# landonclark97/numbotics

Hardware: AMD Instinct MI355X
Metric: collision-checked configs/sec, Kinova 7-DoF + obstacles (higher is better)
Workload: dtype f64

## Files before the change

numbotics_amd/csrc/nbk.hip:

```cpp
#include <hip/hip_runtime.h>
#include <stdint.h>
#include <math.h>
#include <stdio.h>
#include <stdlib.h>
#include <string.h>

#include <memory>
#include <mutex>
#include <atomic>
#include <algorithm>
#include <vector>
#include <string>
#include <map>
#include <dlfcn.h>
#include <hip/hiprtc.h>

#include "../../include/nbk.h"
#include "nbk_device.hpp"
#include "nbk_bf32_common.hpp"

namespace nbk {

struct DevModel {
    int n_q, n_joints, n_rshapes, n_wshapes, n_pairs;
// ... 1138 lines not shown
    const unsigned lo = (unsigned)__builtin_amdgcn_readlane((int)(unsigned)u, l);
    const unsigned hi = (unsigned)__builtin_amdgcn_readlane((int)(unsigned)(u >> 32), l);
    return __builtin_bit_cast(double, ((unsigned long long)hi << 32) | lo);
}

constexpr int NSUB = 256;
constexpr int CNT_TICKET = 1;

struct DevRoute {
    const DevModel& m;
    NBK_DEV int cls(unsigned p) const { return m.vp_cls[p]; }
    NBK_DEV int base(int c) const { return m.cls_base[c]; }
    NBK_DEV int groups(int c) const { return m.cls_groups[c]; }
};
NBK_DEV void flush_items(const DevModel& m, unsigned* lds_queue, int qn, int64_t base_cfg, unsigned long long* q_count,
                         unsigned long long* q_items, unsigned long long cap_sub, int lane, unsigned char* ovf) {
    flush_items_r(DevRoute{m}, lds_queue, qn, base_cfg, q_count, q_items, cap_sub, lane, ovf);
}

__global__ void k_zero_counters(unsigned long long* __restrict__ q_count, unsigned long long* __restrict__ flags, int flag_words) {
    q_count[threadIdx.x * CNT_STRIDE] = 0ull;
    q_count[threadIdx.x * CNT_STRIDE + CNT_TICKET] = 0ull;
    for (int i = threadIdx.x; i < flag_words; i += NSUB) flags[i] = 0ull;
}

NBK_DEV size_t ftab_entries(int W) { return 5 * 256 + 128 + 6 * (size_t)W * 16 + 32 + (size_t)W + 16 + 96 * (size_t)W + 16; }
struct FTab {
    const float *rkey, *rcert, *wkey, *wtc, *wcert, *wcin, *rho, *rneg, *rnd, *wkey2, *wbx;
    const int *rp, *rptri, *wp, *wlist, *n_reach;
};
NBK_DEV FTab ftab_view(const float* tab, int W) {
    const FTabOffsets o = ftab_offsets(W);
// ... 111 lines not shown
        const unsigned long long bal = __builtin_amdgcn_ballot_w64(reach);
        const int wave = t >> 6;
        if ((t & 63) == 0) s_cnt[wave] = __builtin_popcountll(bal);
        __syncthreads();
        int off = s_run;
        for (int i = 0; i < wave; ++i) off += s_cnt[i];
        if (reach) wlist[off + (int)__builtin_amdgcn_mbcnt_hi((unsigned)(bal >> 32), __builtin_amdgcn_mbcnt_lo((unsigned)bal, 0u))] = w;
        __syncthreads();
        if (t == 0) s_run += s_cnt[0] + s_cnt[1] + s_cnt[2] + s_cnt[3];
        __syncthreads();
    }
    if (t == 0) *const_cast<int*>(v.n_reach) = s_run;
}

NBK_DEV void enqueue_bits(const DevModel& m, unsigned long long bits, int jbase, const double* lds_pc, unsigned* lds_queue, int& qn, int lane,
                          int64_t base, unsigned long long* q_count, unsigned long long* q_items, unsigned long long cap, const EdgeSrc& es) {
    while (true) {
        const bool has = bits != 0ull;
        const unsigned long long bal = __builtin_amdgcn_ballot_w64(has);
        if (bal == 0ull) break;
        if (has) {
            const int bit = __builtin_ctzll(bits);
            bits &= bits - 1ull;
            const unsigned long long e0 = __builtin_bit_cast(unsigned long long, lds_pc[4 * (jbase + bit)]);
            const unsigned p = (unsigned)(e0 >> 32) & 0xFFFFFu;
            const int pos = qn + (int)__builtin_amdgcn_mbcnt_hi((unsigned)(bal >> 32), __builtin_amdgcn_mbcnt_lo((unsigned)bal, 0u));
            lds_queue[pos] = (p << 6) | (unsigned)lane;
        }
        qn += __builtin_popcountll(bal);
        if (qn > BQ_CAP - WAVE) { flush_items(m, lds_queue, qn, base, q_count, q_items, cap, lane, es.ovf); qn = 0; }
    }
}


__global__ __launch_bounds__(64) void k_broad(DevModel m, EdgeSrc es, const double* __restrict__ q, int64_t B, double thr,
                                               uint64_t* __restrict__ mask_bits, uint8_t* __restrict__ mask_bytes,
                                               unsigned long long* __restrict__ q_count, unsigned long long* __restrict__ q_items,
                                               unsigned long long cap) {
    extern __shared__ double lds[];
    const int lane = threadIdx.x;
    const int64_t base = (int64_t)blockIdx.x * WAVE;
    const int nq = m.n_q;
    const int P = (NBK_DBG(m) & 2) ? 0 : m.n_pairs;
    double* lds_raw = lds;
    const int qrows = (WAVE * nq * 8 >= BQ_CAP * 4) ? nq : (BQ_CAP * 4 + WAVE * 8 - 1) / (WAVE * 8);
// ... 138 lines not shown
                    hit = hit || (cand && v == 1);
                    bits |= cand ? (1ull << u) : 0ull;
                }
            } else {
                for (int u = 0; u < nn; ++u) {
                    const unsigned long long e0 = __builtin_bit_cast(unsigned long long, pc0[4 * u]);
                    const double key = pc0[4 * u + 1], rhoA = pc0[4 * u + 3];
                    const double* ra = lds_c + (int)(e0 & 0xFFFFull) * WAVE + lane;
                    const double* wc = lds_w + 18 * (int)((e0 >> 16) & 0xFFFFull);
                    const double d[3] = {ra[0] - wc[0], ra[WAVE] - wc[1], ra[2 * WAVE] - wc[2]};
                    const double n[3] = {wc[9], wc[10], wc[11]};
                    bits |= !((dot3(d, n) - rhoA) >= key) ? (1ull << u) : 0ull;
                }
            }
            if (!active || hit || (NBK_DBG(m) & 4)) bits = 0ull;
            enqueue_bits(m, bits, j0 + c0, lds_pc, lds_queue, qn, lane, base, q_count, q_items, cap, es);
        }
        j0 += ncat;
    }
    if (qn > 0) flush_items(m, lds_queue, qn, base, q_count, q_items, cap, lane, es.ovf);
    const unsigned long long word = __builtin_amdgcn_ballot_w64(hit && active);
    if (mask_bits != nullptr && lane == 0) mask_bits[blockIdx.x] = word;
    if (mask_bytes != nullptr && active) mask_bytes[base + lane] = hit ? 1 : 0;
}

template <int S>
__global__ __launch_bounds__(64, 3) void k_broad_reg(DevModel m, EdgeSrc es, const double* __restrict__ q, int64_t B, double thr,
                                                   uint64_t* __restrict__ mask_bits, uint8_t* __restrict__ mask_bytes,
                                                   unsigned long long* __restrict__ q_count, unsigned long long* __restrict__ q_items,
                                                   unsigned long long cap) {
    extern __shared__ double lds[];
    const int lane = threadIdx.x;
    const int64_t base = (int64_t)blockIdx.x * WAVE;
    const int nq = m.n_q;
    const int W = m.n_wshapes;
// ... 122 lines not shown
                bits |= (dot3(d, d) < key) ? (1ull << b) : 0ull;
            }
            if (!active || hit) bits = 0ull;
            while (true) {
                const bool has = bits != 0ull;
                const unsigned long long bal = __builtin_amdgcn_ballot_w64(has);
                if (bal == 0ull) break;
                if (has) {
                    const int bit = __builtin_ctzll(bits);
                    bits &= bits - 1ull;
                    const unsigned p = (unsigned)lds_rp[a * S + bit];
                    const int pos = qn + (int)__builtin_amdgcn_mbcnt_hi((unsigned)(bal >> 32), __builtin_amdgcn_mbcnt_lo((unsigned)bal, 0u));
                    lds_queue[pos] = (p << 6) | (unsigned)lane;
                }
                qn += __builtin_popcountll(bal);
                if (qn > BQ_CAP - WAVE) { flush_items(m, lds_queue, qn, base, q_count, q_items, cap, lane, es.ovf); qn = 0; }
            }
        }
    }
    for (int w = 0; w < W; ++w) {
        const double* wc = m.ws_core + 18 * w;
        const int wk = m.ws_kind[w];
        unsigned long long bits = 0ull;
        if (wk == K_PLANE) {
            const double n[3] = {wc[9], wc[10], wc[11]};
#pragma unroll
            for (int a = 0; a < S; ++a) {
                if (a < m.n_rshapes) {
                    const double key = lds_wkey[w * S + a];
                    const double rhoA = m.rs_core[6 * a + 5];
                    const double d[3] = {cx[a] - wc[0], cy[a] - wc[1], cz[a] - wc[2]};
// ... 30 lines not shown
            }
        }
        if (!active || hit || (NBK_DBG(m) & 4)) bits = 0ull;
        while (true) {
            const bool has = bits != 0ull;
            const unsigned long long bal = __builtin_amdgcn_ballot_w64(has);
            if (bal == 0ull) break;
            if (has) {
                const int bit = __builtin_ctzll(bits);
                bits &= bits - 1ull;
                const unsigned p = (unsigned)lds_wp[w * S + bit];
                const int pos = qn + (int)__builtin_amdgcn_mbcnt_hi((unsigned)(bal >> 32), __builtin_amdgcn_mbcnt_lo((unsigned)bal, 0u));
                lds_queue[pos] = (p << 6) | (unsigned)lane;
            }
            qn += __builtin_popcountll(bal);
            if (qn > BQ_CAP - WAVE) { flush_items(m, lds_queue, qn, base, q_count, q_items, cap, lane, es.ovf); qn = 0; }
        }
    }
    if (qn > 0) flush_items(m, lds_queue, qn, base, q_count, q_items, cap, lane, es.ovf);
    const unsigned long long word = __builtin_amdgcn_ballot_w64(hit && active);
    if (mask_bits != nullptr && lane == 0) mask_bits[blockIdx.x] = word;
    if (mask_bytes != nullptr && active) mask_bytes[base + lane] = hit ? 1 : 0;
}

struct XfF { float R[9]; float t[3]; };


template <int KZ>
NBK_DEV void joint_apply_axis_f(const float* M, const float* toff, const XfF& P, float s, float c, XfF& o) {
    constexpr int U = (KZ + 1) % 3, V = (KZ + 2) % 3;
    float Lu[3], Lv[3];
#pragma unroll
    for (int r = 0; r < 3; ++r) {
        Lu[r] = __builtin_fmaf(s, M[18 + 3 * r + U], -c * M[9 + 3 * r + U]);
// ... 250 lines not shown
        const float* tab_rnd = ft.rnd;
        const float* tab_wkey2 = ft.wkey2;
#define NBK_ENQUEUE(cond_, pidx_)                                                                                               \
        {                                                                                                                       \
            const bool c_ = (cond_);                                                                                            \
            const unsigned long long cm_ = __builtin_amdgcn_ballot_w64(c_);                                                     \
            if (cm_ != 0ull) {                                                                                                  \
                if (c_) {                                                                                                       \
                    const int pos_ = qn + (int)__builtin_amdgcn_mbcnt_hi((unsigned)(cm_ >> 32), __builtin_amdgcn_mbcnt_lo((unsigned)cm_, 0u)); \
                    lds_queue[pos_] = ((unsigned)(pidx_) << 6) | (unsigned)lane;                                                \
                }                                                                                                               \
                qn += __builtin_popcountll(cm_);                                                                                \
            }                                                                                                                   \
        }
#define NBK_ROOM(slots_)                                                                                                        \
        if (qn > qcap - (slots_) * WAVE) { flush_items(m, lds_queue, qn, base, q_count, q_items, cap, lane, es.ovf); qn = 0; }
#if defined(NBK_BF32_ABL) && NBK_BF32_ABL == 5
        for (int wi = 0; wi < (e2 == 12345.0f ? n_reach : 0); ++wi) {
#else
        for (int wi = 0; wi < n_reach; ++wi) {
#endif
            const int w = ft.wlist[wi];
            const float* wc = m.f_tab + m.f_wc + 18 * w;
            const int wk = m.ws_kind[w];
            const Row16f wkey2r = *reinterpret_cast<const Row16f*>(tab_wkey2 + w * 16);
            const Row16f wcertr = *reinterpret_cast<const Row16f*>(tab_wcert + w * 16);
            const Row16f wkeyr = *reinterpret_cast<const Row16f*>(tab_wkey + w * 16);
            bool c[S];
            bool ch = false;
#pragma unroll
            for (int a = 0; a < S; ++a) c[a] = false;
// ... 132 lines not shown
                    }
                    hit = hit || (acc_f < 0);
                    const bool live = active && !hit;
                    NBK_ROOM(S)
#pragma unroll
                    for (int b = a + 1; b < S; ++b) {
                        const V2i ei = __builtin_bit_cast(V2i, ev[b / 2]);
                        NBK_ENQUEUE(((b % 2) ? ei.y : ei.x) < 0 && live, ft.rp[a * 16 + b]);
                    }
                }
            }
        }
#undef NBK_ENQUEUE
#undef NBK_ROOM
        NBK_BSTAMP(4);
        if (qn > 0) flush_items(m, lds_queue, qn, base, q_count, q_items, cap, lane, es.ovf);
        const unsigned long long word = __builtin_amdgcn_ballot_w64(hit && active);
        if (mask_bits != nullptr && lane == 0) mask_bits[blockIdx.x] = word;
        if (mask_bytes != nullptr && active) mask_bytes[base + lane] = hit ? 1 : 0;
#ifdef NBK_BF32_STAMP
        NBK_BSTAMP(5);
        if (lane == 0) { unsigned long long* pr_ = g_broad_prof + 8 * (blockIdx.x & 16383u); for (int e_ = 0; e_ < 5; ++e_) pr_[e_] += bstamp[e_ + 1] - bstamp[e_]; pr_[7] += 1ull; }
#endif
        return;
    }
    const bool cert_ok = e2 <= m.f_e2max;
    bool certh = false;
    for (int wi = 0; wi < n_reach; ++wi) {
        const int w = ft.wlist[wi];
        const float* wc = m.f_tab + m.f_wc + 18 * w;
        const int wk = m.ws_kind[w];
// ... 73 lines not shown
        }
        hit = hit || (cert_ok && certh);
        if (!active || hit || (NBK_DBG(m) & 4)) bits = 0ull;
        while (true) {
            const bool has = bits != 0ull;
            const unsigned long long bal = __builtin_amdgcn_ballot_w64(has);
            if (bal == 0ull) break;
            if (has) {
                const int bit = __builtin_ctzll(bits);
                bits &= bits - 1ull;
                const unsigned p = (unsigned)tab_wp[w * 16 + bit];
                const int pos = qn + (int)__builtin_amdgcn_mbcnt_hi((unsigned)(bal >> 32), __builtin_amdgcn_mbcnt_lo((unsigned)bal, 0u));
                lds_queue[pos] = (p << 6) | (unsigned)lane;
            }
            qn += __builtin_popcountll(bal);
            if (qn > BQ_CAP - WAVE) { flush_items(m, lds_queue, qn, base, q_count, q_items, cap, lane, es.ovf); qn = 0; }
        }
    }
    if (m.bq_count[1] > 0) {
#pragma unroll
        for (int a = 0; a < S - 1; ++a) {
            unsigned long long bits = 0ull;
#pragma unroll
            for (int b = a + 1; b < S; ++b) {
                const float rs = tab_rkey[a * 16 + b];
                const float r = rs + e2;
                const float dx = cx(a) - cx(b), dy = cy(a) - cy(b), dz = cz(a) - cz(b);
                const float dd = __builtin_fmaf(dz, dz, __builtin_fmaf(dy, dy, dx * dx));
                bits |= (rs >= 0.0f && dd < r * r * up) ? (1ull << b) : 0ull;
                certh = certh || (dd < tab_rcert[a * 16 + b]);
            }
            hit = hit || (cert_ok && certh);
            if (!active || hit) bits = 0ull;
            while (true) {
                const bool has = bits != 0ull;
                const unsigned long long bal = __builtin_amdgcn_ballot_w64(has);
                if (bal == 0ull) break;
                if (has) {
                    const int bit = __builtin_ctzll(bits);
                    bits &= bits - 1ull;
                    const unsigned p = (unsigned)ft.rp[a * 16 + bit];
                    const int pos = qn + (int)__builtin_amdgcn_mbcnt_hi((unsigned)(bal >> 32), __builtin_amdgcn_mbcnt_lo((unsigned)bal, 0u));
                    lds_queue[pos] = (p << 6) | (unsigned)lane;
                }
                qn += __builtin_popcountll(bal);
                if (qn > BQ_CAP - WAVE) { flush_items(m, lds_queue, qn, base, q_count, q_items, cap, lane, es.ovf); qn = 0; }
            }
        }
    }
    if (qn > 0) flush_items(m, lds_queue, qn, base, q_count, q_items, cap, lane, es.ovf);
    const unsigned long long word = __builtin_amdgcn_ballot_w64(hit && active);
    if (mask_bits != nullptr && lane == 0) mask_bits[blockIdx.x] = word;
    if (mask_bytes != nullptr && active) mask_bytes[base + lane] = hit ? 1 : 0;
}
#undef cx
#undef cy
#undef cz
#undef cx2v
#undef cy2v
#undef cz2v

NBK_DEV void build_core(const DevModel& m, int ref, const Xf& T, Core& o) {
    const bool robot = ref >= 0;
    const int w = robot ? 0 : ~ref;
    const double* wc = m.ws_core + 18 * w;
// ... 20 lines not shown
}

constexpr int NARROW_T = 64;
constexpr int HULL_LDS_MAX = 16 * 1024;
static inline size_t narrow_hull_lds(int hull_blob_n) { return (hull_blob_n > 0 && (size_t)hull_blob_n * 8 <= (size_t)HULL_LDS_MAX) ? (size_t)hull_blob_n * 8 : 0; }
#ifndef NARROW_WAVES_GEN
#define NARROW_WAVES_GEN 2
#endif
constexpr int NARROW_WAVES_BOOL = 2;

NBK_DEV void mark_hit(long long b, uint64_t* mask_bits, uint8_t* mask_bytes) {
    if (mask_bits != nullptr) atomicOr(reinterpret_cast<unsigned long long*>(mask_bits) + (b >> 6), 1ull << (b & 63));
    if (mask_bytes != nullptr) mask_bytes[b] = 1;
}

#ifndef NBK_WALK_BRANCHED
#define NBK_WALK_BRANCHED 0
#endif
template <int INFL, int KA, int KB>
NBK_DEV void narrow_walk(GjkBool& gb, const Core& A, const Core& Bc, double tc, bool& have, bool& hard, long long b,
                         uint64_t* mask_bits, uint8_t* mask_bytes, unsigned& trips) {
    constexpr bool STRAIGHT = !NBK_WALK_BRANCHED && (INFL == 0 || INFL == 1) && (KA == K_BOX || KA == K_CYL) && (KB == K_BOX || KB == K_CYL);
    if constexpr (STRAIGHT) {
        bool hit = false;
        int r = gjkb_step_sl<INFL, KA, KB, true>(gb, A, Bc, tc);
        while (true) {
            trips += 1u;
            hit = hit || (have && r == 2);
            hard = hard || (have && r == 3);
            have = have && r == 0;
            if (__builtin_amdgcn_ballot_w64(have) == 0ull) break;
            r = gjkb_step_sl<INFL, KA, KB, false>(gb, A, Bc, tc);
        }
        if (hit) mark_hit(b, mask_bits, mask_bytes);
    } else {
        while (__builtin_amdgcn_ballot_w64(have) != 0ull) {
            trips += 1u;
            if (have) {
                const int r = gjkb_step_k<INFL, KA, KB>(gb, A, Bc, tc);
                if (r != 0) { if (r == 2) mark_hit(b, mask_bits, mask_bytes); hard = hard || r == 3; have = false; }
            }
        }
    }
}

template <int INFL>
NBK_DEV void narrow_walk_any(GjkBool& gb, const Core& A, const Core& Bc, double tc, bool& have, bool& hard, long long b,
                             uint64_t* mask_bits, uint8_t* mask_bytes, unsigned& trips) {
    const unsigned long long walkers = __builtin_amdgcn_ballot_w64(have);
    if (walkers == 0ull) return;
    const int l0 = __builtin_ctzll(walkers);
// ... 44 lines not shown
    unsigned long long* ticket = q_count + sub * CNT_STRIDE + CNT_TICKET;
    double* hull_lds = qstage + NARROW_T * m.n_q;
    const bool hull_staged = m.hull_blob_n > 0 && m.hull_blob_n * 8 <= HULL_LDS_MAX;
    if (hull_staged && (unsigned long long)part * NARROW_T < n) {
        for (int i = threadIdx.x; i < m.hull_blob_n; i += NARROW_T) hull_lds[i] = m.hull_blob[i];
        __syncthreads();
    }
    for (unsigned long long chunk = part; chunk * NARROW_T < n; ) {
        const unsigned long long i0 = chunk * NARROW_T;
        unsigned next_ticket = 0u;
        unsigned trips = 0u;
        if (threadIdx.x == 0) next_ticket = (unsigned)atomicAdd(ticket, 1ull);
        chunk = nparts;
        {
            const unsigned long long i = i0 + threadIdx.x;
            const bool live = i < n;
            unsigned long long item = 0;
            if (i == i_first) item = item_first;
            else if (live) item = __hip_atomic_load(q_items + i, __ATOMIC_RELAXED, __HIP_MEMORY_SCOPE_AGENT);
            if (!live) item = 0;
            const long long b = (long long)(item >> 20);
            const int p = (int)(item & 0xFFFFFull);
            NBK_STAMP(1);
            const int4 info = m.vp_info[p];
            const int ra = live ? info.x : -1, rb = live ? info.y : -1;
            const unsigned ma = live ? (unsigned)info.z : 0u, mb = live ? (unsigned)info.w : 0u;
            Xf TA, TB;
            xf_from12(m.base_pose, TA);
            TB = TA;
            double* myq = qstage + threadIdx.x * m.n_q;
            const int nq1 = m.n_q - 1;
            if (es.map != nullptr) {
                unsigned e;
                const double et = edge_t(es, es.map[b], e);
                const double eomt = 1.0 - et;
                const double* sp = es.starts + (size_t)e * m.n_q;
                const double* gp = es.goals + (size_t)e * m.n_q;
                for (int j0 = 0; j0 < m.n_q; j0 += 4) {
                    double sv[4], gv[4];
#pragma unroll
                    for (int u = 0; u < 4; ++u) { const int j = (j0 + u) < nq1 ? (j0 + u) : nq1; sv[u] = sp[j]; gv[u] = gp[j]; }
#pragma unroll
                    for (int u = 0; u < 4; ++u)
                        if (j0 + u <= nq1) { const double a = eomt * sv[u]; const double bb = et * gv[u]; myq[j0 + u] = a + bb; }
                }
            } else {
                const double* qrow = q + b * m.n_q;
                for (int j0 = 0; j0 < m.n_q; j0 += 8) {
                    double qv[8];
#pragma unroll
                    for (int u = 0; u < 8; ++u) { const int j = (j0 + u) < nq1 ? (j0 + u) : nq1; qv[u] = qrow[j]; }
#pragma unroll
                    for (int u = 0; u < 8; ++u)
                        if (j0 + u <= nq1) myq[j0 + u] = qv[u];
                }
            }
            NBK_STAMP(2);
            for (int k = 0; k < ((NBK_DBG(m) & 16) ? 0 : m.n_joints); ++k) {
                const bool in_a = (ma >> k) & 1u, in_b = (mb >> k) & 1u;
                if (__builtin_amdgcn_ballot_w64(in_a || in_b) == 0ull) continue;
                if (in_a || in_b) {
                    const double qk = myq[m.joint_qidx[k]];
                    Xf nxt;
                    joint_apply(m, k, in_a ? TA : TB, qk, nxt);
                    if (in_a) TA = nxt;
                    if (in_b) TB = nxt;
                }
            }
            NBK_STAMP(3);
            bool pooled = false;
            Core A, Bc;
// ... 39 lines not shown
            bool have = pooled && !(NBK_DBG(m) & 8);
            if constexpr (MODE == 1) {
                GjkBool gb;
                gjkb_init(gb, A, Bc);
                bool hard = false;
                narrow_walk_any<0>(gb, A, Bc, tc, have, hard, b, mask_bits, mask_bytes, trips);
            } else if constexpr (MODE == 3) {
                GjkBool gb;
                gjkb_init(gb, A, Bc);
                bool hard = have && (A.kind == K_HULL || Bc.kind == K_HULL);
                have = have && !hard;
                narrow_walk_any<2>(gb, A, Bc, tc, have, hard, b, mask_bits, mask_bytes, trips);
                if (__builtin_amdgcn_ballot_w64(hard) != 0ull) {
                    GjkPred g;
                    gjk_pred_init(g, A, Bc);
                    while (__builtin_amdgcn_ballot_w64(hard) != 0ull) {
                        if (hard) {
                            const int r = gjk_pred_step<true>(g, A, Bc, tc);
                            if (r != 0) { if (r == 2) mark_hit(b, mask_bits, mask_bytes); hard = false; }
                        }
                    }
                }
            } else if constexpr (MODE == 2) {
                GjkPred g;
                gjk_pred_init(g, A, Bc);
                while (__builtin_amdgcn_ballot_w64(have) != 0ull) {
                    if (have) {
                        const int r = gjk_pred_step(g, A, Bc, tc);
                        if (r != 0) { if (r == 2) mark_hit(b, mask_bits, mask_bytes); have = false; }
                    }
                }
            } else {
                GjkBool gb;
                GjkPred g;
                gjkb_init(gb, A, Bc);
                gjk_pred_init(g, A, Bc);
                bool walk = tc >= 0.0 && A.kind != K_HULL && Bc.kind != K_HULL;
                while (__builtin_amdgcn_ballot_w64(have) != 0ull) {
                    if (have) {
                        const int r = walk ? gjkb_step<2>(gb, A, Bc, tc) : gjk_pred_step(g, A, Bc, tc);
                        if (r == 3) walk = false;
                        else if (r != 0) { if (r == 2) mark_hit(b, mask_bits, mask_bytes); have = false; }
                    }
                }
            }
        }
        __syncthreads();
        chunk += (unsigned)__builtin_amdgcn_readfirstlane((int)next_ticket);
        if (prof && i0 == (unsigned long long)part * NARROW_T) {
            NBK_STAMP(6);
            if (threadIdx.x == 0) {
                for (int e = 0; e < 6; ++e) atomicAdd(&g_narrow_prof[e], stamp[e + 1] - stamp[e]);
                atomicAdd(&g_narrow_prof[6], (unsigned long long)trips);
// ... 1908 lines not shown
    for (StreamWs* w : m->wss) delete w;
    if (m->scalar_q) (void)hipHostFree(m->scalar_q);
    if (m->scalar_out) (void)hipHostFree(m->scalar_out);
    if (m->scalar_stream) (void)hipStreamDestroy(m->scalar_stream);
    if (m->world_ev) (void)hipEventDestroy(m->world_ev);
    if (m->world_stage) (void)hipHostFree(m->world_stage);
    delete m;
}

extern "C" int32_t nbk_debug_narrow_profile(unsigned long long* out, int32_t reset) {
    if (out != nullptr) NBK_HIP(hipMemcpyFromSymbol(out, HIP_SYMBOL(nbk::g_narrow_prof), sizeof(unsigned long long) * 16));
    if (reset) { unsigned long long z[16] = {0}; z[13] = ~0ull; NBK_HIP(hipMemcpyToSymbol(HIP_SYMBOL(nbk::g_narrow_prof), z, sizeof(z))); }
    return NBK_OK;
}

extern "C" int32_t nbk_debug_broad_profile(unsigned long long* out, int32_t reset) {
#ifdef NBK_BF32_STAMP
    static std::vector<unsigned long long> h(16384 * 8);
    if (out != nullptr) {
        NBK_HIP(hipMemcpyFromSymbol(h.data(), HIP_SYMBOL(nbk::g_broad_prof), sizeof(unsigned long long) * h.size()));
        for (int e = 0; e < 8; ++e) { out[e] = 0; for (size_t b = 0; b < 16384; ++b) out[e] += h[8 * b + e]; }
    }
    if (reset) { std::fill(h.begin(), h.end(), 0ull); NBK_HIP(hipMemcpyToSymbol(HIP_SYMBOL(nbk::g_broad_prof), h.data(), sizeof(unsigned long long) * h.size())); }
    return NBK_OK;
#else
    (void)out; (void)reset;
    return NBK_ERR_UNSUPPORTED;
#endif
}

// ... 1174 lines not shown
```

numbotics_amd/csrc/nbk_bf32_common.hpp:

```cpp
#ifndef NBK_BF32_COMMON_HPP
#define NBK_BF32_COMMON_HPP

#define NBK_BF32_DEV __device__ __forceinline__

namespace nbk {

constexpr int WAVE = 64;
constexpr int BQ_CAP = 512;
constexpr int CNT_STRIDE = 16;

typedef float V2f __attribute__((ext_vector_type(2)));
typedef int V2i __attribute__((ext_vector_type(2)));
struct alignas(64) Row16f { float v[16]; };

struct FTabOffsets { int rkey, rp, rcert, rptri, rneg, rnd, wkey, wtc, wp, wcert, wcin, wkey2, rho, n_reach, wlist, wbx; };
__host__ __device__ constexpr FTabOffsets ftab_offsets(int W) {
    const int w16 = W * 16;
    const int wkey = 1408, wtc = wkey + w16, rho = wtc + 5 * w16, n_reach = rho + 32, wlist = n_reach + 16;
    return FTabOffsets{0, 256, 512, 768, 896, 1152, wkey, wtc, wtc + w16, wtc + 2 * w16, wtc + 3 * w16, wtc + 4 * w16, rho, n_reach, wlist,
                       wlist + ((W + 15) & ~15)};
}

NBK_BF32_DEV V2f splat2(float x) { return V2f{x, x}; }
NBK_BF32_DEV V2f fma2(V2f a, V2f b, V2f c) { return __builtin_elementwise_fma(a, b, c); }
// ... 145 lines not shown
        }
        const float rr = ((tc > 0.0f ? tc : 0.0f) + rho) + e2;
        if (ex2 >= rr * rr * up) cand = false;
    }
    certh = certh || (dd < cert);
    return cand;
}
NBK_BF32_DEV bool robot_slot_gen(float dx, float dy, float dz, float rs, float e2, float cert, bool& certh) {
    const float up = 1.0f + 2.4e-7f;
    const float r = rs + e2;
    const float dd = __builtin_fmaf(dz, dz, __builtin_fmaf(dy, dy, dx * dx));
    certh = certh || (dd < cert);
    return rs >= 0.0f && dd < r * r * up;
}

template <class Route>
NBK_BF32_DEV void flush_items_r(const Route& rt, unsigned* lds_queue, int qn, long long base_cfg, unsigned long long* q_count,
                                unsigned long long* q_items, unsigned long long cap_sub, int lane, unsigned char* ovf) {
    __syncthreads();
    for (int i0 = 0; i0 < qn; i0 += WAVE) {
        const int i = i0 + lane;
        const bool has = i < qn;
        const unsigned it = has ? lds_queue[i] : 0u;
        const int cls = has ? rt.cls(it >> 6) : 0;
        unsigned long long bc[4];
#pragma unroll
        for (int c = 0; c < 4; ++c) bc[c] = __builtin_amdgcn_ballot_w64(has && cls == c);
        const unsigned long long mine_cnt = lane == 0 ? bc[0] : (lane == 1 ? bc[1] : (lane == 2 ? bc[2] : bc[3]));
        unsigned long long off = 0;
        if (lane < 4 && mine_cnt != 0ull)
            off = atomicAdd(q_count + (unsigned long long)(rt.base(lane) + (int)(blockIdx.x % (unsigned)rt.groups(lane))) * CNT_STRIDE,
                            (unsigned long long)__builtin_popcountll(mine_cnt));
        const unsigned olo = (unsigned)__builtin_amdgcn_ds_bpermute(cls * 4, (int)(unsigned)off);
        const unsigned ohi = (unsigned)__builtin_amdgcn_ds_bpermute(cls * 4, (int)(unsigned)(off >> 32));
        if (has) {
            const unsigned long long mb_ = cls == 0 ? bc[0] : (cls == 1 ? bc[1] : (cls == 2 ? bc[2] : bc[3]));
            const unsigned long long slot = (((unsigned long long)ohi << 32) | olo) +
                                            __builtin_amdgcn_mbcnt_hi((unsigned)(mb_ >> 32), __builtin_amdgcn_mbcnt_lo((unsigned)mb_, 0u));
// ... 13 lines not shown
```

numbotics_amd/csrc/nbk_bf32_spec.hpp:

```cpp

#define NBK_SPEC_DEV __device__ __forceinline__
#define NBK_SPEC_INLINE __attribute__((always_inline))

namespace nbk_spec {

using namespace nbk;
enum { K_BOX = 2, K_HULL = 4, K_PLANE = 5 };
enum { JK_PRISMATIC = 4 };

template <int V> struct IC { static constexpr int value = V; };
template <int B, int E, class F> NBK_SPEC_DEV void sfor(F&& f) {
    if constexpr (B < E) { f(IC<B>{}); sfor<B + 1, E>(f); }
}

template <class Spec> struct SpecRoute {
    const int* __restrict__ vp_cls;
    NBK_SPEC_DEV int cls(unsigned p) const { return vp_cls[p]; }
    NBK_SPEC_DEV int base(int c) const { return Spec::cls_base[c]; }
    NBK_SPEC_DEV int groups(int c) const { return Spec::cls_groups[c]; }
};

template <class Spec>
NBK_SPEC_DEV void broad_f32_spec(const double* __restrict__ q, long long B, const float* __restrict__ ftb, const float* __restrict__ tab,
                                 unsigned long long* __restrict__ mask_bits, unsigned char* __restrict__ mask_bytes,
// ... 71 lines not shown
    __syncthreads();
    int qn = 0;
#define NBK_SPEC_ENQUEUE(cond_, pidx_)                                                                                          \
    {                                                                                                                           \
        const bool c_ = (cond_);                                                                                                \
        const unsigned long long cm_ = __builtin_amdgcn_ballot_w64(c_);                                                         \
        if (cm_ != 0ull) {                                                                                                      \
            if (c_) {                                                                                                           \
                const int pos_ = qn + (int)__builtin_amdgcn_mbcnt_hi((unsigned)(cm_ >> 32), __builtin_amdgcn_mbcnt_lo((unsigned)cm_, 0u)); \
                lds_queue[pos_] = ((unsigned)(pidx_) << 6) | (unsigned)lane;                                                    \
            }                                                                                                                   \
            qn += __builtin_popcountll(cm_);                                                                                    \
        }                                                                                                                       \
    }
#define NBK_SPEC_ROOM(slots_)                                                                                                   \
    if (qn > qcap - (slots_) * WAVE) { flush_items_r(SpecRoute<Spec>{vp_cls}, lds_queue, qn, base, q_count, q_items, cap, lane, ovf); qn = 0; }
    const float* wbx_all = tab + FO.wbx;
    if (__builtin_amdgcn_ballot_w64(!(e2 <= Spec::f_e2max)) == 0ull) {
        sfor<0, Spec::NW>([&](auto WI) NBK_SPEC_INLINE {
            constexpr int wi = decltype(WI)::value;
            constexpr int w = Spec::wl[wi];
            constexpr int wk = Spec::wk[wi];
            const float* wc = ftb + Spec::f_wc + 18 * w;
            if constexpr (wk == K_BOX || wk == K_HULL) {
                const float* wb = wbx_all + w * 96;
                const float* ob = ftb + Spec::f_wobb + 6 * w;
                int cwv[SB];
                int acc_c = 0, acc_h = 0;
                sfor<0, SB / 2>([&](auto I) NBK_SPEC_INLINE {
                    constexpr int i = decltype(I)::value;
                    cwv[2 * i] = 0; cwv[2 * i + 1] = 0;
// ... 98 lines not shown
        const int* tab_rp = reinterpret_cast<const int*>(tab + FO.rp);
        const float* tab_rkey = tab + FO.rkey; const float* tab_rcert = tab + FO.rcert;
        auto drain = [&](unsigned long long bits, const int* ptab) NBK_SPEC_INLINE {
            while (true) {
                const bool has = bits != 0ull;
                const unsigned long long bal = __builtin_amdgcn_ballot_w64(has);
                if (bal == 0ull) break;
                if (has) {
                    const int bit = __builtin_ctzll(bits);
                    bits &= bits - 1ull;
                    const unsigned p = (unsigned)ptab[bit];
                    const int pos = qn + (int)__builtin_amdgcn_mbcnt_hi((unsigned)(bal >> 32), __builtin_amdgcn_mbcnt_lo((unsigned)bal, 0u));
                    lds_queue[pos] = (p << 6) | (unsigned)lane;
                }
                qn += __builtin_popcountll(bal);
                if (qn > BQ_CAP - WAVE) { flush_items_r(SpecRoute<Spec>{vp_cls}, lds_queue, qn, base, q_count, q_items, cap, lane, ovf); qn = 0; }
            }
        };
        sfor<0, Spec::NW>([&](auto WI) NBK_SPEC_INLINE {
            constexpr int wi = decltype(WI)::value;
            constexpr int w = Spec::wl[wi];
            constexpr int wk = Spec::wk[wi];
            const float* wc = ftb + Spec::f_wc + 18 * w;
            unsigned long long bits = 0ull;
            sfor<0, S>([&](auto A) NBK_SPEC_INLINE {
                constexpr int a = decltype(A)::value;
                if constexpr (Spec::wpair(wi, a) >= 0) {
                    const float dx = cxa[a] - wc[0], dy = cya[a] - wc[1], dz = cza[a] - wc[2];
                    if constexpr (wk == K_PLANE) {
                        if (tab_wp[w * 16 + a] >= 0)
                            bits |= plane_slot_gen(dx, dy, dz, wc, tab_wkey[w * 16 + a], tab_rho[a], e2, tab_wcert[w * 16 + a], certh) ? (1ull << a) : 0ull;
// ... 19 lines not shown
                sfor<a + 1, S>([&](auto Bb) NBK_SPEC_INLINE {
                    constexpr int b = decltype(Bb)::value;
                    if constexpr (Spec::rr_p(a, b) >= 0) {
                        bits |= robot_slot_gen(cxa[a] - cxa[b], cya[a] - cya[b], cza[a] - cza[b], tab_rkey[a * 16 + b], e2, tab_rcert[a * 16 + b], certh)
                                    ? (1ull << b) : 0ull;
                    }
                });
                hit = hit || (cert_ok && certh);
                if (!active || hit) bits = 0ull;
                drain(bits, tab_rp + a * 16);
            });
        }
    }
#undef NBK_SPEC_ENQUEUE
#undef NBK_SPEC_ROOM
    if (qn > 0) flush_items_r(SpecRoute<Spec>{vp_cls}, lds_queue, qn, base, q_count, q_items, cap, lane, ovf);
    const unsigned long long word = __builtin_amdgcn_ballot_w64(hit && active);
    if (mask_bits != nullptr && lane == 0) mask_bits[blockIdx.x] = word;
    if (mask_bytes != nullptr && active) mask_bytes[base + lane] = hit ? 1 : 0;
}

}

#ifndef NBK_SPEC_WAVES
#define NBK_SPEC_WAVES 5
#endif
extern "C" __global__ __launch_bounds__(64, NBK_SPEC_WAVES) void k_broad_f32_spec(
        const double* __restrict__ q, long long B, const float* __restrict__ ftb, const float* __restrict__ tab,
        unsigned long long* __restrict__ mask_bits, unsigned char* __restrict__ mask_bytes, unsigned long long* __restrict__ q_count,
        unsigned long long* __restrict__ q_items, unsigned long long cap, unsigned char* ovf, const int* __restrict__ vp_cls) {
    nbk_spec::broad_f32_spec<Spec>(q, B, ftb, tab, mask_bits, mask_bytes, q_count, q_items, cap, ovf, vp_cls);
// ... 2 lines not shown
```

Before: 9.410 billion.

## Skip queued narrow-phase work for configs already marked colliding

When the broad phase flushes candidate pairs, it now drops entries whose configuration already has a hit in the current wave. The narrow phase reads the collision mask before transforms, so pairs for configs another pair already marked as colliding go inactive. The GJK loops also re-poll the mask periodically so lanes can exit early. This cuts redundant narrow-phase work for colliding configs, at the cost of extra atomic global loads and ballot logic in hot loops. A debug queue-count API is added too.

```diff
diff --git a/numbotics_amd/csrc/nbk.hip b/numbotics_amd/csrc/nbk.hip
--- a/numbotics_amd/csrc/nbk.hip
+++ b/numbotics_amd/csrc/nbk.hip
@@ -1176,8 +1176,8 @@
     NBK_DEV int groups(int c) const { return m.cls_groups[c]; }
 };
 NBK_DEV void flush_items(const DevModel& m, unsigned* lds_queue, int qn, int64_t base_cfg, unsigned long long* q_count,
-                         unsigned long long* q_items, unsigned long long cap_sub, int lane, unsigned char* ovf) {
-    flush_items_r(DevRoute{m}, lds_queue, qn, base_cfg, q_count, q_items, cap_sub, lane, ovf);
+                         unsigned long long* q_items, unsigned long long cap_sub, int lane, unsigned char* ovf, unsigned long long dead) {
+    flush_items_r(DevRoute{m}, lds_queue, qn, base_cfg, q_count, q_items, cap_sub, lane, ovf, dead);
 }
 
 __global__ void k_zero_counters(unsigned long long* __restrict__ q_count, unsigned long long* __restrict__ flags, int flag_words) {
@@ -1319,7 +1319,7 @@
 }
 
 NBK_DEV void enqueue_bits(const DevModel& m, unsigned long long bits, int jbase, const double* lds_pc, unsigned* lds_queue, int& qn, int lane,
-                          int64_t base, unsigned long long* q_count, unsigned long long* q_items, unsigned long long cap, const EdgeSrc& es) {
+                          int64_t base, unsigned long long* q_count, unsigned long long* q_items, unsigned long long cap, const EdgeSrc& es, bool hit) {
     while (true) {
         const bool has = bits != 0ull;
         const unsigned long long bal = __builtin_amdgcn_ballot_w64(has);
@@ -1333,7 +1333,7 @@
             lds_queue[pos] = (p << 6) | (unsigned)lane;
         }
         qn += __builtin_popcountll(bal);
-        if (qn > BQ_CAP - WAVE) { flush_items(m, lds_queue, qn, base, q_count, q_items, cap, lane, es.ovf); qn = 0; }
+        if (qn > BQ_CAP - WAVE) { flush_items(m, lds_queue, qn, base, q_count, q_items, cap, lane, es.ovf, __builtin_amdgcn_ballot_w64(hit)); qn = 0; }
     }
 }
 
@@ -1502,11 +1502,11 @@
                 }
             }
             if (!active || hit || (NBK_DBG(m) & 4)) bits = 0ull;
-            enqueue_bits(m, bits, j0 + c0, lds_pc, lds_queue, qn, lane, base, q_count, q_items, cap, es);
+            enqueue_bits(m, bits, j0 + c0, lds_pc, lds_queue, qn, lane, base, q_count, q_items, cap, es, hit);
         }
         j0 += ncat;
     }
-    if (qn > 0) flush_items(m, lds_queue, qn, base, q_count, q_items, cap, lane, es.ovf);
+    if (qn > 0) flush_items(m, lds_queue, qn, base, q_count, q_items, cap, lane, es.ovf, __builtin_amdgcn_ballot_w64(hit));
     const unsigned long long word = __builtin_amdgcn_ballot_w64(hit && active);
     if (mask_bits != nullptr && lane == 0) mask_bits[blockIdx.x] = word;
     if (mask_bytes != nullptr && active) mask_bytes[base + lane] = hit ? 1 : 0;
@@ -1659,7 +1659,7 @@
                     lds_queue[pos] = (p << 6) | (unsigned)lane;
                 }
                 qn += __builtin_popcountll(bal);
-                if (qn > BQ_CAP - WAVE) { flush_items(m, lds_queue, qn, base, q_count, q_items, cap, lane, es.ovf); qn = 0; }
+                if (qn > BQ_CAP - WAVE) { flush_items(m, lds_queue, qn, base, q_count, q_items, cap, lane, es.ovf, __builtin_amdgcn_ballot_w64(hit)); qn = 0; }
             }
         }
     }
@@ -1720,10 +1720,10 @@
                 lds_queue[pos] = (p << 6) | (unsigned)lane;
             }
             qn += __builtin_popcountll(bal);
-            if (qn > BQ_CAP - WAVE) { flush_items(m, lds_queue, qn, base, q_count, q_items, cap, lane, es.ovf); qn = 0; }
-        }
-    }
-    if (qn > 0) flush_items(m, lds_queue, qn, base, q_count, q_items, cap, lane, es.ovf);
+            if (qn > BQ_CAP - WAVE) { flush_items(m, lds_queue, qn, base, q_count, q_items, cap, lane, es.ovf, __builtin_amdgcn_ballot_w64(hit)); qn = 0; }
+        }
+    }
+    if (qn > 0) flush_items(m, lds_queue, qn, base, q_count, q_items, cap, lane, es.ovf, __builtin_amdgcn_ballot_w64(hit));
     const unsigned long long word = __builtin_amdgcn_ballot_w64(hit && active);
     if (mask_bits != nullptr && lane == 0) mask_bits[blockIdx.x] = word;
     if (mask_bytes != nullptr && active) mask_bytes[base + lane] = hit ? 1 : 0;
@@ -2004,7 +2004,7 @@
             }                                                                                                                   \
         }
 #define NBK_ROOM(slots_)                                                                                                        \
-        if (qn > qcap - (slots_) * WAVE) { flush_items(m, lds_queue, qn, base, q_count, q_items, cap, lane, es.ovf); qn = 0; }
+        if (qn > qcap - (slots_) * WAVE) { flush_items(m, lds_queue, qn, base, q_count, q_items, cap, lane, es.ovf, __builtin_amdgcn_ballot_w64(hit)); qn = 0; }
 #if defined(NBK_BF32_ABL) && NBK_BF32_ABL == 5
         for (int wi = 0; wi < (e2 == 12345.0f ? n_reach : 0); ++wi) {
 #else
@@ -2167,7 +2167,7 @@
 #undef NBK_ENQUEUE
 #undef NBK_ROOM
         NBK_BSTAMP(4);
-        if (qn > 0) flush_items(m, lds_queue, qn, base, q_count, q_items, cap, lane, es.ovf);
+        if (qn > 0) flush_items(m, lds_queue, qn, base, q_count, q_items, cap, lane, es.ovf, __builtin_amdgcn_ballot_w64(hit));
         const unsigned long long word = __builtin_amdgcn_ballot_w64(hit && active);
         if (mask_bits != nullptr && lane == 0) mask_bits[blockIdx.x] = word;
         if (mask_bytes != nullptr && active) mask_bytes[base + lane] = hit ? 1 : 0;
@@ -2271,7 +2271,7 @@
                 lds_queue[pos] = (p << 6) | (unsigned)lane;
             }
             qn += __builtin_popcountll(bal);
-            if (qn > BQ_CAP - WAVE) { flush_items(m, lds_queue, qn, base, q_count, q_items, cap, lane, es.ovf); qn = 0; }
+            if (qn > BQ_CAP - WAVE) { flush_items(m, lds_queue, qn, base, q_count, q_items, cap, lane, es.ovf, __builtin_amdgcn_ballot_w64(hit)); qn = 0; }
         }
     }
     if (m.bq_count[1] > 0) {
@@ -2301,11 +2301,11 @@
                     lds_queue[pos] = (p << 6) | (unsigned)lane;
                 }
                 qn += __builtin_popcountll(bal);
-                if (qn > BQ_CAP - WAVE) { flush_items(m, lds_queue, qn, base, q_count, q_items, cap, lane, es.ovf); qn = 0; }
-            }
-        }
-    }
-    if (qn > 0) flush_items(m, lds_queue, qn, base, q_count, q_items, cap, lane, es.ovf);
+                if (qn > BQ_CAP - WAVE) { flush_items(m, lds_queue, qn, base, q_count, q_items, cap, lane, es.ovf, __builtin_amdgcn_ballot_w64(hit)); qn = 0; }
+            }
+        }
+    }
+    if (qn > 0) flush_items(m, lds_queue, qn, base, q_count, q_items, cap, lane, es.ovf, __builtin_amdgcn_ballot_w64(hit));
     const unsigned long long word = __builtin_amdgcn_ballot_w64(hit && active);
     if (mask_bits != nullptr && lane == 0) mask_bits[blockIdx.x] = word;
     if (mask_bytes != nullptr && active) mask_bytes[base + lane] = hit ? 1 : 0;
@@ -2356,6 +2356,43 @@
     if (mask_bytes != nullptr) mask_bytes[b] = 1;
 }
 
+#ifndef NBK_MOOT_P1
+#define NBK_MOOT_P1 1
+#endif
+#ifndef NBK_MOOT_WALK
+#define NBK_MOOT_WALK 1
+#endif
+#ifndef NBK_MOOT_N0
+#define NBK_MOOT_N0 6
+#endif
+#ifndef NBK_MOOT_N
+#define NBK_MOOT_N 2
+#endif
+NBK_DEV unsigned long long moot_load(long long b, const uint64_t* mask_bits, const uint8_t* mask_bytes) {
+    if (mask_bits != nullptr)
+        return __hip_atomic_load(reinterpret_cast<const unsigned long long*>(mask_bits) + (b >> 6), __ATOMIC_RELAXED, __HIP_MEMORY_SCOPE_AGENT);
+    if (mask_bytes != nullptr) return (unsigned long long)__hip_atomic_load(mask_bytes + b, __ATOMIC_RELAXED, __HIP_MEMORY_SCOPE_AGENT);
+    return 0ull;
+}
+NBK_DEV bool moot_bit(unsigned long long w, long long b, const uint64_t* mask_bits) {
+    return mask_bits != nullptr ? ((w >> (b & 63)) & 1ull) != 0ull : w != 0ull;
+}
+
+struct MootPoll {
+    unsigned long long w = 0ull;
+    unsigned t;
+    NBK_DEV explicit MootPoll(unsigned steps_done) : t(steps_done) {}
+    NBK_DEV bool poll(long long b, const uint64_t* mask_bits, const uint8_t* mask_bytes) {
+        bool dead = false;
+        if (NBK_MOOT_WALK) {
+            if (t > NBK_MOOT_N0 && (t - 1u - NBK_MOOT_N0) % NBK_MOOT_N == 0u) dead = moot_bit(w, b, mask_bits);
+            if (t >= NBK_MOOT_N0 && (t - NBK_MOOT_N0) % NBK_MOOT_N == 0u) w = moot_load(b, mask_bits, mask_bytes);
+            t += 1u;
+        }
+        return dead;
+    }
+};
+
 #ifndef NBK_WALK_BRANCHED
 #define NBK_WALK_BRANCHED 0
 #endif
@@ -2365,18 +2402,24 @@
     constexpr bool STRAIGHT = !NBK_WALK_BRANCHED && (INFL == 0 || INFL == 1) && (KA == K_BOX || KA == K_CYL) && (KB == K_BOX || KB == K_CYL);
     if constexpr (STRAIGHT) {
         bool hit = false;
+        MootPoll mp(1u);
         int r = gjkb_step_sl<INFL, KA, KB, true>(gb, A, Bc, tc);
         while (true) {
             trips += 1u;
             hit = hit || (have && r == 2);
             hard = hard || (have && r == 3);
-            have = have && r == 0;
+            const bool moot = mp.poll(b, mask_bits, mask_bytes);
+            have = have && r == 0 && !moot;
             if (__builtin_amdgcn_ballot_w64(have) == 0ull) break;
             r = gjkb_step_sl<INFL, KA, KB, false>(gb, A, Bc, tc);
         }
         if (hit) mark_hit(b, mask_bits, mask_bytes);
     } else {
-        while (__builtin_amdgcn_ballot_w64(have) != 0ull) {
+        MootPoll mp(0u);
+        while (true) {
+            const bool moot = mp.poll(b, mask_bits, mask_bytes);
+            have = have && !moot;
+            if (__builtin_amdgcn_ballot_w64(have) == 0ull) break;
             trips += 1u;
             if (have) {
                 const int r = gjkb_step_k<INFL, KA, KB>(gb, A, Bc, tc);
@@ -2451,17 +2494,16 @@
         chunk = nparts;
         {
             const unsigned long long i = i0 + threadIdx.x;
-            const bool live = i < n;
+            const bool queued = i < n;
             unsigned long long item = 0;
             if (i == i_first) item = item_first;
-            else if (live) item = __hip_atomic_load(q_items + i, __ATOMIC_RELAXED, __HIP_MEMORY_SCOPE_AGENT);
-            if (!live) item = 0;
+            else if (queued) item = __hip_atomic_load(q_items + i, __ATOMIC_RELAXED, __HIP_MEMORY_SCOPE_AGENT);
+            if (!queued) item = 0;
             const long long b = (long long)(item >> 20);
             const int p = (int)(item & 0xFFFFFull);
             NBK_STAMP(1);
+            const unsigned long long mword = NBK_MOOT_P1 ? moot_load(b, mask_bits, mask_bytes) : 0ull;
             const int4 info = m.vp_info[p];
-            const int ra = live ? info.x : -1, rb = live ? info.y : -1;
-            const unsigned ma = live ? (unsigned)info.z : 0u, mb = live ? (unsigned)info.w : 0u;
             Xf TA, TB;
             xf_from12(m.base_pose, TA);
             TB = TA;
@@ -2492,6 +2534,9 @@
                         if (j0 + u <= nq1) myq[j0 + u] = qv[u];
                 }
             }
+            const bool live = queued && !moot_bit(mword, b, mask_bits);
+            const int ra = live ? info.x : -1, rb = live ? info.y : -1;
+            const unsigned ma = live ? (unsigned)info.z : 0u, mb = live ? (unsigned)info.w : 0u;
             NBK_STAMP(2);
             for (int k = 0; k < ((NBK_DBG(m) & 16) ? 0 : m.n_joints); ++k) {
                 const bool in_a = (ma >> k) & 1u, in_b = (mb >> k) & 1u;
@@ -2561,7 +2606,11 @@
                 if (__builtin_amdgcn_ballot_w64(hard) != 0ull) {
                     GjkPred g;
                     gjk_pred_init(g, A, Bc);
-                    while (__builtin_amdgcn_ballot_w64(hard) != 0ull) {
+                    MootPoll mp(0u);
+                    while (true) {
+                        const bool moot = mp.poll(b, mask_bits, mask_bytes);
+                        hard = hard && !moot;
+                        if (__builtin_amdgcn_ballot_w64(hard) == 0ull) break;
                         if (hard) {
                             const int r = gjk_pred_step<true>(g, A, Bc, tc);
                             if (r != 0) { if (r == 2) mark_hit(b, mask_bits, mask_bytes); hard = false; }
@@ -2571,7 +2620,11 @@
             } else if constexpr (MODE == 2) {
                 GjkPred g;
                 gjk_pred_init(g, A, Bc);
-                while (__builtin_amdgcn_ballot_w64(have) != 0ull) {
+                MootPoll mp(0u);
+                while (true) {
+                    const bool moot = mp.poll(b, mask_bits, mask_bytes);
+                    have = have && !moot;
+                    if (__builtin_amdgcn_ballot_w64(have) == 0ull) break;
                     if (have) {
                         const int r = gjk_pred_step(g, A, Bc, tc);
                         if (r != 0) { if (r == 2) mark_hit(b, mask_bits, mask_bytes); have = false; }
@@ -2583,7 +2636,11 @@
                 gjkb_init(gb, A, Bc);
                 gjk_pred_init(g, A, Bc);
                 bool walk = tc >= 0.0 && A.kind != K_HULL && Bc.kind != K_HULL;
-                while (__builtin_amdgcn_ballot_w64(have) != 0ull) {
+                MootPoll mp(0u);
+                while (true) {
+                    const bool moot = mp.poll(b, mask_bits, mask_bytes);
+                    have = have && !moot;
+                    if (__builtin_amdgcn_ballot_w64(have) == 0ull) break;
                     if (have) {
                         const int r = walk ? gjkb_step<2>(gb, A, Bc, tc) : gjk_pred_step(g, A, Bc, tc);
                         if (r == 3) walk = false;
@@ -4522,6 +4579,25 @@
     return NBK_OK;
 }
 
+extern "C" int32_t nbk_debug_queue_items(const nbk_model* m, unsigned long long* out) {
+    if (m == nullptr || out == nullptr) return NBK_ERR_INVALID;
+    NBK_HIP(hipDeviceSynchronize());
+    nbk_model* mm = const_cast<nbk_model*>(m);
+    std::lock_guard<std::mutex> lock(mm->mu);
+    std::vector<unsigned long long> h((size_t)NSUB * CNT_STRIDE);
+    out[0] = out[1] = out[2] = 0ull;
+    for (StreamWs* w : mm->wss) {
+        if (w->ws == nullptr || w->epoch == 0u) continue;
+        const size_t set = w->ready ? (size_t)((w->epoch - 1u) & 1u) : 0;
+        NBK_HIP(hipMemcpy(h.data(), static_cast<unsigned long long*>(w->ws) + set * NSUB * CNT_STRIDE, h.size() * sizeof(unsigned long long), hipMemcpyDeviceToHost));
+        for (int sub = 0; sub < NSUB; ++sub) {
+            const unsigned long long c = h[(size_t)sub * CNT_STRIDE];
+            out[0] += c; out[1] += (c + NARROW_T - 1) / NARROW_T; out[2] += c != 0ull;
+        }
+    }
+    return NBK_OK;
+}
+
 extern "C" int32_t nbk_debug_broad_profile(unsigned long long* out, int32_t reset) {
 #ifdef NBK_BF32_STAMP
     static std::vector<unsigned long long> h(16384 * 8);
diff --git a/numbotics_amd/csrc/nbk_bf32_common.hpp b/numbotics_amd/csrc/nbk_bf32_common.hpp
--- a/numbotics_amd/csrc/nbk_bf32_common.hpp
+++ b/numbotics_amd/csrc/nbk_bf32_common.hpp
@@ -183,14 +183,18 @@
     return rs >= 0.0f && dd < r * r * up;
 }
 
+#ifndef NBK_MOOT_FLUSH
+#define NBK_MOOT_FLUSH 1
+#endif
 template <class Route>
 NBK_BF32_DEV void flush_items_r(const Route& rt, unsigned* lds_queue, int qn, long long base_cfg, unsigned long long* q_count,
-                                unsigned long long* q_items, unsigned long long cap_sub, int lane, unsigned char* ovf) {
+                                unsigned long long* q_items, unsigned long long cap_sub, int lane, unsigned char* ovf,
+                                unsigned long long dead) {
     __syncthreads();
     for (int i0 = 0; i0 < qn; i0 += WAVE) {
         const int i = i0 + lane;
-        const bool has = i < qn;
-        const unsigned it = has ? lds_queue[i] : 0u;
+        const unsigned it = i < qn ? lds_queue[i] : 0u;
+        const bool has = i < qn && !(NBK_MOOT_FLUSH && ((dead >> (it & 63u)) & 1ull));
         const int cls = has ? rt.cls(it >> 6) : 0;
         unsigned long long bc[4];
 #pragma unroll
diff --git a/numbotics_amd/csrc/nbk_bf32_spec.hpp b/numbotics_amd/csrc/nbk_bf32_spec.hpp
--- a/numbotics_amd/csrc/nbk_bf32_spec.hpp
+++ b/numbotics_amd/csrc/nbk_bf32_spec.hpp
@@ -109,7 +109,7 @@
         }                                                                                                                       \
     }
 #define NBK_SPEC_ROOM(slots_)                                                                                                   \
-    if (qn > qcap - (slots_) * WAVE) { flush_items_r(SpecRoute<Spec>{vp_cls}, lds_queue, qn, base, q_count, q_items, cap, lane, ovf); qn = 0; }
+    if (qn > qcap - (slots_) * WAVE) { flush_items_r(SpecRoute<Spec>{vp_cls}, lds_queue, qn, base, q_count, q_items, cap, lane, ovf, __builtin_amdgcn_ballot_w64(hit != 0)); qn = 0; }
     const float* wbx_all = tab + FO.wbx;
     if (__builtin_amdgcn_ballot_w64(!(e2 <= Spec::f_e2max)) == 0ull) {
         sfor<0, Spec::NW>([&](auto WI) NBK_SPEC_INLINE {
@@ -238,7 +238,7 @@
                     lds_queue[pos] = (p << 6) | (unsigned)lane;
                 }
                 qn += __builtin_popcountll(bal);
-                if (qn > BQ_CAP - WAVE) { flush_items_r(SpecRoute<Spec>{vp_cls}, lds_queue, qn, base, q_count, q_items, cap, lane, ovf); qn = 0; }
+                if (qn > BQ_CAP - WAVE) { flush_items_r(SpecRoute<Spec>{vp_cls}, lds_queue, qn, base, q_count, q_items, cap, lane, ovf, __builtin_amdgcn_ballot_w64(hit != 0)); qn = 0; }
             }
         };
         sfor<0, Spec::NW>([&](auto WI) NBK_SPEC_INLINE {
@@ -288,7 +288,7 @@
     }
 #undef NBK_SPEC_ENQUEUE
 #undef NBK_SPEC_ROOM
-    if (qn > 0) flush_items_r(SpecRoute<Spec>{vp_cls}, lds_queue, qn, base, q_count, q_items, cap, lane, ovf);
+    if (qn > 0) flush_items_r(SpecRoute<Spec>{vp_cls}, lds_queue, qn, base, q_count, q_items, cap, lane, ovf, __builtin_amdgcn_ballot_w64(hit != 0));
     const unsigned long long word = __builtin_amdgcn_ballot_w64(hit && active);
     if (mask_bits != nullptr && lane == 0) mask_bits[blockIdx.x] = word;
     if (mask_bytes != nullptr && active) mask_bytes[base + lane] = hit ? 1 : 0;
```

Result: slower. 9.125 billion (-3.0%).
